# SeanNaren/deepspeech.pytorch

Hardware: NVIDIA H100
Metric: utterances/sec (train step, 161x1000 spectrogram) (higher is better)
Workload: dtype fp16-operands(rnn)+tf32(conv/fc)

## Files before the change

deepspeech.pytorch_b200/csrc/rnn_persistent_tc.cu:

```cuda
#include <cooperative_groups.h>
#include <cuda_fp16.h>
#include <dlfcn.h>
#include <stdlib.h>

#include "common.cuh"
#include "rnn_cells.cuh"
#include "rnn_common.cuh"
#include "tc_common.cuh"

namespace cg = cooperative_groups;

namespace ds2 {

namespace rp {
constexpr int UT = 16;
constexpr int MM = 64;
constexpr int BK = 32;
constexpr int STAGES = 8;
constexpr int THREADS = 288;
constexpr int A_BYTES = MM * 128;
constexpr long long SPIN_LIMIT = 4000000000LL;
}

struct PersistParams {
// ... 711 lines not shown
      uint32_t ph = 0;
      for (int step = 1; step < T; ++step) {
        const int t = d == 0 ? T - 1 - step : step;
        const int tn = d == 0 ? t + 1 : t - 1;
        for (int c = 0; c < NK; ++c) {
          mbar_wait(&empty[s], ph ^ 1);
          mbar_arrive_expect_tx(&full[s], tx_bytes);
          tma_load_2d(smem + s * STAGE_BYTES, &p.tmW[d], &full[s], c * BK, u0);
          if (c == 0) {
            grid_wait_counter(ctr, (unsigned int)p.NT * (unsigned int)step, p.err);
            fence_proxy_async_global();
            trace_stamp(p.trace, p.T, step, 0);
          }
          const int k0 = c * BK;
          if (RNN == DS2_RNN_GRU && k0 >= 2 * H)
            tma_load_2d(smem + s * STAGE_BYTES + A_BYTES, &p.tmV2[d], &full[s], k0 - 2 * H, tn * B);
          else
            tma_load_2d(smem + s * STAGE_BYTES + A_BYTES, &p.tmV[d], &full[s], d * GH + k0, tn * B);
          if (++s == STAGES) { s = 0; ph ^= 1; }
        }
      }
    }
  } else if (warp >= 4) {
    with_nch<4>(NB, [&](auto nch) {
      WgAcc<1, decltype(nch)::value> acc;
      {
        const uint64_t a_base = smem_desc_sw128(smem_u32(smem));
        const uint64_t b_base = smem_desc_sw128(smem_u32(smem + A_BYTES));
        const uint64_t stage_step = (uint64_t)(STAGE_BYTES >> 4);
        int s = 0;
        uint32_t ph = 0;
        for (int step = 1; step < T; ++step) {
          for (int c = 0; c < NK; ++c) {
            mbar_wait(&full[s], ph);
            if (c == 0 && lane == 0) trace_stamp(p.trace, p.T, step, 1);
            if (c == NK - 1 && lane == 0) trace_stamp(p.trace, p.T, step, 2);
            const uint64_t ad = a_base + (uint64_t)s * stage_step, bd = b_base + (uint64_t)s * stage_step;
            wg_mma4<false>(acc, ad, bd, c > 0);
            wg_release_all(&empty[s]);
            if (++s == STAGES) { s = 0; ph ^= 1; }
          }
          wg_publish(acc, acc_img, accum_bar);
        }
      }
    });
  } else {
    const int q = warp % 4;
    const int e = threadIdx.x;
    uint32_t acc_phase = 0;
    for (int step = 0; step < T; ++step) {
      const int t = d == 0 ? T - 1 - step : step;
      const int tp = d == 0 ? t - 1 : t + 1;
      const bool tp_in = tp >= 0 && tp < T;
      if (q == 0 && step > 0) {
        mbar_wait(accum_bar, acc_phase);
        if (lane == 0) trace_stamp(p.trace, p.T, step, 3);
        for (int cb = 0; cb < NB; cb += 32) {
          float acc[32];
          tmem_ld32(acc_img, acc_pitch(NB), (uint32_t)cb, acc);
          if (lane < UT) {
#pragma unroll
            for (int j = 0; j < 32; ++j)
              if (cb + j < B) ex[lane * NBp + cb + j] = acc[j];
          }
        }
      }
      if (step > 0) acc_phase ^= 1;
      named_bar_sync(1, 128);
      if (e == 0) trace_stamp(p.trace, p.T, step, 4);
      for (int pi = e; pi < UT * B; pi += 128) {
        const int ui = pi % UT, b = pi / UT;
        const bool valid = t < p.len[b];
        const bool pin = tp_in && (d == 0 || tp < p.len[b]);
        const size_t si = (((size_t)d * T + t) * B + b) * H + u0 + ui;
        const size_t sp = (((size_t)d * T + (tp_in ? tp : 0)) * B + b) * H + u0 + ui;
        float* gp = p.gates + (((size_t)t * B + b) * D + d) * GH + u0 + ui;
        if (!valid) {
#pragma unroll
          for (int g = 0; g < G; ++g) gp[g * H] = 0.f;
          if (RNN == DS2_RNN_GRU) p.aux[si] = 0.f;
        } else {
          float dh = p.dy[((size_t)t * B + b) * H + u0 + ui] + ex[ui * NBp + b];
          if (RNN == DS2_RNN_LSTM) {
            const float c_prev = pin ? p.aux[sp] : 0.f;
            LstmBwd r = lstm_cell_bwd(gp[0], gp[H], gp[2 * H], gp[3 * H], p.aux[si], c_prev, dh, cst[ui * NBp + b]);
            gp[0] = r.di; gp[H] = r.df; gp[2 * H] = r.dg; gp[3 * H] = r.d_o;
            cst[ui * NBp + b] = r.dc_prev;
          } else if (RNN == DS2_RNN_GRU) {
            const float h_prev = pin ? p.hseq[sp] : 0.f;
            dh += cst[ui * NBp + b];
            GruBwd r = gru_cell_bwd(gp[0], gp[H], gp[2 * H], p.aux[si], h_prev, dh);
            gp[0] = r.dr; gp[H] = r.dz; gp[2 * H] = r.dxn;
            p.aux[si] = r.dhn;
            cst[ui * NBp + b] = r.dh_prev;
          } else {
            const float h = p.hseq[si];
            gp[0] = dh * (1.f - h * h);
          }
        }
      }
      named_bar_sync(1, 128);
      if (e == 0) {
        fence_proxy_async_global();
        red_release(ctr, 1u);
        trace_stamp(p.trace, p.T, step, 5);
      }
    }
  }
  __syncthreads();
}

__device__ __forceinline__ uint32_t mapa_u32(uint32_t addr, uint32_t rank) {
  uint32_t r;
  asm volatile("mapa.shared::cluster.u32 %0, %1, %2;" : "=r"(r) : "r"(addr), "r"(rank));
  return r;
}
__device__ __forceinline__ float ld_dsmem(uint32_t addr) {
  float v;
  asm volatile("ld.shared::cluster.f32 %0, [%1];" : "=f"(v) : "r"(addr) : "memory");
  return v;
}
__device__ __forceinline__ void mbar_arrive_remote(uint32_t cluster_addr) {
  asm volatile("mbarrier.arrive.release.cluster.shared::cluster.b64 _, [%0];" ::"r"(cluster_addr) : "memory");
}
__device__ __forceinline__ void mbar_wait_cluster(uint64_t* bar, uint32_t parity, int* err) {
  uint32_t ok = 0, it = 0;
  long long t0 = 0;
  while (!ok) {
    asm volatile(
        "{\n\t.reg .pred p;\n\t"
        "mbarrier.try_wait.parity.acquire.cluster.shared::cta.b64 p, [%1], %2;\n\t"
        "selp.u32 %0, 1, 0, p;\n\t}"
        : "=r"(ok)
        : "r"(tc::smem_u32(bar)), "r"(parity)
        : "memory");
    if (!ok && (++it & 1023u) == 0) {
      if (t0 == 0) t0 = clock64();
      if (*(volatile int*)err) return;
      if (clock64() - t0 > rp::SPIN_LIMIT) { *(volatile int*)err = 1; return; }
    }
  }
}
__host__ __device__ constexpr int xt_cgs(int rows) { return (rows + rows / 8) * 4 + 4; }
__host__ __device__ constexpr int xt_slice(int rows, int nb) { return (nb / 4) * xt_cgs(rows); }
__device__ __forceinline__ int xt_off(int rows, int row, int col) {
  return (col >> 2) * xt_cgs(rows) + (row + (row >> 3)) * 4 + (col & 3);
}
__device__ __forceinline__ void st_async_v4(uint32_t cluster_addr, float a, float b, float c, float d, uint32_t cluster_bar) {
  asm volatile("st.async.weak.shared::cluster.mbarrier::complete_tx::bytes.v4.f32 [%0], {%1, %2, %3, %4}, [%5];" ::"r"(
                   cluster_addr),
               "f"(a), "f"(b), "f"(c), "f"(d), "r"(cluster_bar)
               : "memory");
}
__device__ __forceinline__ void bulk_load(void* smem_dst, const void* src, uint32_t bytes, uint64_t* bar) {
  asm volatile("cp.async.bulk.shared::cluster.global.mbarrier::complete_tx::bytes [%0], [%1], %2, [%3];" ::"r"(
                   tc::smem_u32(smem_dst)),
               "l"(src), "r"(bytes), "r"(tc::smem_u32(bar))
               : "memory");
}
__device__ __forceinline__ void cluster_sync_all() {
  asm volatile("barrier.cluster.arrive.release.aligned;\n\tbarrier.cluster.wait.acquire.aligned;" ::: "memory");
}

__device__ __forceinline__ __half to_half_sat(float v) {
  return __float2half_rn(fminf(fmaxf(v, -65000.f), 65000.f));
}
__device__ __forceinline__ int pow2_exp_for(unsigned int m_bits, int sx_prev) {
  if (m_bits == 0u || m_bits >= 0x7f800000u) return sx_prev;
  const int E = (int)((m_bits >> 23) & 0xffu);
  return max(-100, min(100, 134 - E));
}
__device__ __forceinline__ float pow2f(int ex) { return __int_as_float((ex + 127) << 23); }

template <int RNN, bool RES, int CL, int NKR_T = 0, bool XG = false>
__global__ void __launch_bounds__(rp::THREADS, 1) rnn_bwd_splitk_kernel(const __grid_constant__ PersistParams p) {
  using namespace rp;
  using namespace tc;
  static_assert(!XG || (RES && CL == 4), "the L2 exchange is built for the resident 4-CTA variant");
  constexpr int G = RNN == DS2_RNN_LSTM ? 4 : (RNN == DS2_RNN_GRU ? 3 : 1);
  constexpr int UM = UT * CL;
  constexpr int A_BYTES = UM * 128;
  extern __shared__ uint8_t smem_raw[];
  uint8_t* smem = smem_raw + ((1024u - (tc::smem_u32(smem_raw) & 1023u)) & 1023u);
  const int NB = p.NB, B = p.B, T = p.T, H = p.H, D = p.D;
  const int B_BYTES = NB * 128, STAGE_BYTES = A_BYTES + B_BYTES;
  const int NBp = NB + 1;
  const int NKR = NKR_T ? NKR_T : (G * H / CL) / 64;
  const int NG = grp_count(NKR);
  const int ring_bytes = RES ? NKR * STAGE_BYTES : STAGES * STAGE_BYTES;
  float* part = reinterpret_cast<float*>(smem + ring_bytes);
  float* cst = part + CL * xt_slice(UT, NB);
  int* lens_s = reinterpret_cast<int*>(cst + UT * NBp);
  unsigned int* cta_max = reinterpret_cast<unsigned int*>(lens_s + ((NB + 1) & ~1));
  uint64_t* full = reinterpret_cast<uint64_t*>(cta_max + 2);
  uint64_t* empty = full + (RES ? 32 : STAGES);
  uint64_t* accum_bar = empty + STAGES;
  uint64_t* part_bar = accum_bar + 1;
  float* acc_img = reinterpret_cast<float*>(part_bar + 1);

  const int warp = threadIdx.x / 32, lane = threadIdx.x % 32;
  const int ks = blockIdx.x % CL;
  const int cl = blockIdx.x / CL;
  const int NTc = H / UM;
  const int d = p.d0 + cl / NTc, ut = cl % NTc;
  const int GH = G * H;
  const int Kc = GH / CL, NK = Kc / BK;
  const int kbase = ks * Kc;
  const int u0 = ut * UM + ks * UT;
  unsigned int* ctr = p.bar + 32 * d;
  const unsigned int n_arrive = (unsigned int)(NTc * CL);
  const int ss = xt_slice(UT, NB);
  const int grp0 = (d * NTc + ut) * CL;
  auto xslot = [&](int cta, int src, int step) { return p.xbuf + ((size_t)(cta * CL + src) * 2 + (step & 1)) * ss; };

  if (warp == 0 && lane == 0) {
    tma_prefetch_desc(&p.tmW[d]);
    tma_prefetch_desc(&p.tmV[d]);
    for (int i = 0; i < (RES ? 32 : STAGES); ++i) mbar_init(&full[i], 1);
    for (int i = 0; i < STAGES; ++i) mbar_init(&empty[i], RES ? 1 : 128);
    mbar_init(accum_bar, 1);
    mbar_init(part_bar, XG ? 2 : 1);
    fence_barrier_init();
    cta_max[0] = 0u;
  }
  for (int i = threadIdx.x; i < UT * NBp; i += THREADS) cst[i] = 0.f;
  for (int i = threadIdx.x; i < NB; i += THREADS) lens_s[i] = i < B ? p.len[i] : 0;
  __syncthreads();
  if constexpr (!XG) cluster_sync_all();
  const uint32_t tx_bytes = (uint32_t)(UM * 128 + B * 128);

  if (warp == 8) {
    if (RES) {
      if (lane == 0) {
        mbar_arrive_expect_tx(&empty[0], (uint32_t)(NKR * UM * 128));
        for (int c = 0; c < NKR; ++c) tma_load_2d(smem + c * A_BYTES, &p.tmW[d], &empty[0], kbase + c * 64, ut * UM);
        uint8_t* vbuf = smem + NKR * A_BYTES;
        for (int step = 1; step < T; ++step) {
          const int t = d == 0 ? T - 1 - step : step;
          const int tn = d == 0 ? t + 1 : t - 1;
          grid_wait_counter(ctr, n_arrive * (unsigned int)step, p.err);
          fence_proxy_async_global();
          trace_stamp(p.trace, p.T, step, 0);
          const unsigned int gm = ld_relaxed(p.gmax + (size_t)d * (T + 1) + step);
          for (int g = 0; g < NG; ++g) {
            uint64_t* fb = full + g;
            const int c0 = grp_begin(g), c1 = min(NKR, grp_begin(g + 1));
            if (c1 == NKR) *(volatile unsigned int*)(cta_max + 1) = gm;
            if (p.box3) {
              mbar_arrive_expect_tx(fb, (uint32_t)(4 * B_BYTES));
              tma_load_3d(vbuf + c0 * B_BYTES, &p.tmV3[d], fb, 0, tn * B, (d * GH + kbase) / 64 + c0);
            } else {
              mbar_arrive_expect_tx(fb, (uint32_t)((c1 - c0) * B * 128));
              for (int c = c0; c < c1; ++c)
                tma_load_2d(vbuf + c * B_BYTES, &p.tmV[d], fb, d * GH + kbase + c * 64, tn * B);
            }
          }
          trace_stamp(p.trace, p.T, step, 1);
          if constexpr (XG) {
            grid_wait_counter(p.xcnt + grp0 + ks, (unsigned int)((CL - 1) * step), p.err);
            fence_proxy_async_global();
            mbar_arrive_expect_tx(part_bar, (uint32_t)((CL - 1) * ss * 4));
            for (int src = 0; src < CL; ++src)
              if (src != ks) bulk_load(part + src * ss, xslot(grp0 + ks, src, step), (uint32_t)(ss * 4), part_bar);
          }
        }
      }
    } else
    if (lane == 0) {
      int s = 0;
      uint32_t ph = 0;
      for (int step = 1; step < T; ++step) {
        const int t = d == 0 ? T - 1 - step : step;
        const int tn = d == 0 ? t + 1 : t - 1;
        for (int c = 0; c < NK; ++c) {
          mbar_wait(&empty[s], ph ^ 1);
          mbar_arrive_expect_tx(&full[s], tx_bytes);
          const int k0 = kbase + c * BK;
          tma_load_2d(smem + s * STAGE_BYTES, &p.tmW[d], &full[s], k0, ut * UM);
          if (c == 0) {
            grid_wait_counter(ctr, n_arrive * (unsigned int)step, p.err);
            fence_proxy_async_global();
            trace_stamp(p.trace, p.T, step, 0);
          }
          if (RNN == DS2_RNN_GRU && k0 >= 2 * H)
            tma_load_2d(smem + s * STAGE_BYTES + A_BYTES, &p.tmV2[d], &full[s], k0 - 2 * H, tn * B);
          else
            tma_load_2d(smem + s * STAGE_BYTES + A_BYTES, &p.tmV[d], &full[s], d * GH + k0, tn * B);
          if (++s == STAGES) { s = 0; ph ^= 1; }
        }
      }
    }
  } else if (warp >= 4) {
    with_nch<UM == 64 ? 4 : 2>(NB, [&](auto nch) {
      WgAcc<UM / 64, decltype(nch)::value> acc;
      if (RES) {
        {
          const uint64_t a_base = warp_uniform(smem_desc_sw128(smem_u32(smem)));
          const uint64_t b_base = warp_uniform(smem_desc_sw128(smem_u32(smem + NKR * A_BYTES)));
          const uint64_t a_step = (uint64_t)(A_BYTES >> 4), b_step = (uint64_t)(B_BYTES >> 4);
          mbar_wait(&empty[0], 0);
          uint32_t ph = 0;
          for (int step = 1; step < T; ++step) {
            if constexpr (NKR_T > 0) {
              constexpr int NGT = (NKR_T + 3) / 4;
  #pragma unroll
              for (int g = 0; g < NGT; ++g) {
                mbar_wait(full + g, ph);
                if (g == 0 && lane == 0) trace_stamp(p.trace, p.T, step, 2);
                if (g == NGT - 1 && lane == 0) trace_stamp(p.trace, p.T, step, 3);
  #pragma unroll
                for (int c = 4 * g; c < (4 * g + 4 < NKR_T ? 4 * g + 4 : NKR_T); ++c) {
                  const uint64_t ad = a_base + (uint64_t)c * a_step, bd = b_base + (uint64_t)c * b_step;
                  wg_mma4<true>(acc, ad, bd, c > 0);
                }
              }
            } else {
              for (int g = 0; g < NG; ++g) {
                mbar_wait(full + g, ph);
                if (g == 0 && lane == 0) trace_stamp(p.trace, p.T, step, 2);
                const int c0 = grp_begin(g), c1 = min(NKR, grp_begin(g + 1));
                if (c1 == NKR && lane == 0) trace_stamp(p.trace, p.T, step, 3);
                for (int c = c0; c < c1; ++c) {
                  const uint64_t ad = a_base + (uint64_t)c * a_step, bd = b_base + (uint64_t)c * b_step;
                  wg_mma4<true>(acc, ad, bd, c > 0);
                }
              }
            }
            wg_publish(acc, acc_img, accum_bar);
            if (lane == 0) trace_stamp(p.trace, p.T, step, 4);
            ph ^= 1;
          }
        }
      } else
      {
        const uint64_t a_base = smem_desc_sw128(smem_u32(smem));
        const uint64_t b_base = smem_desc_sw128(smem_u32(smem + A_BYTES));
        const uint64_t stage_step = (uint64_t)(STAGE_BYTES >> 4);
        int s = 0;
        uint32_t ph = 0;
        for (int step = 1; step < T; ++step) {
          for (int c = 0; c < NK; ++c) {
            mbar_wait(&full[s], ph);
            if (c == 0 && lane == 0) trace_stamp(p.trace, p.T, step, 1);
            if (c == NK - 1 && lane == 0) trace_stamp(p.trace, p.T, step, 2);
            const uint64_t ad = a_base + (uint64_t)s * stage_step, bd = b_base + (uint64_t)s * stage_step;
            wg_mma4<false>(acc, ad, bd, c > 0);
            wg_release_all(&empty[s]);
            if (++s == STAGES) { s = 0; ph ^= 1; }
          }
          wg_publish(acc, acc_img, accum_bar);
        }
      }
    });
  } else {
    const int q = warp % 4;
    const int e = threadIdx.x;
    const int ul = lane & 15, half = lane >> 4;
    uint32_t acc_phase = 0, part_phase = 0;
    const int dst_cta = CL == 4 ? q : 2 * q + half;
    const uint32_t dst_row = XG ? 0u : mapa_u32(smem_u32(part), (uint32_t)dst_cta) + (uint32_t)(ks * ss * 4);
    const uint32_t dst_bar = XG ? 0u : mapa_u32(smem_u32(part_bar), (uint32_t)dst_cta);
    const uint32_t part_tx = (uint32_t)(CL * UT * NB * 4);
    float bsum[5][4];
#pragma unroll
    for (int i = 0; i < 5; ++i)
#pragma unroll
      for (int j = 0; j < 4; ++j) bsum[i][j] = 0.f;
    int sx_prev = 0, sx_cur = 0;
    if (RES) sx_cur = pow2_exp_for(__ldg(p.dymax + (d == 0 ? T - 1 : 0)), 0);
    float s_cur = pow2f(sx_cur), inv_prev = 1.f;
    const float nscale = (RES && p.dgn16) ? __ldg(p.nscale) : 1.f;
    for (int step = 0; step < T; ++step) {
      const int t = d == 0 ? T - 1 - step : step;
      const int tp = d == 0 ? t - 1 : t + 1;
      const bool tp_in = tp >= 0 && tp < T;
      float lmax = 0.f;
      const unsigned int dym = RES ? __ldg(p.dymax + t) : 0u;
      constexpr int NPF = 4;
      const bool single = B <= 32;
      const int uq = 4 * (e & 3), b_own = e >> 2;
      auto ld4 = [](const float* src, float (&v)[NPF]) {
        const float4 x = *reinterpret_cast<const float4*>(src);
        v[0] = x.x; v[1] = x.y; v[2] = x.z; v[3] = x.w;
      };
      auto load_coefs = [&](int b, float (&k)[6][NPF], float (&dyv)[NPF], bool& valid) {
#pragma unroll
        for (int i = 0; i < 6; ++i)
#pragma unroll
          for (int j = 0; j < NPF; ++j) k[i][j] = 0.f;
#pragma unroll
        for (int j = 0; j < NPF; ++j) dyv[j] = 0.f;
        valid = b < B && t < lens_s[b < B ? b : 0];
        if (!valid) return;
        const bool pin = tp_in && (d == 0 || tp < lens_s[b]);
        const size_t si = (((size_t)d * T + t) * B + b) * H + u0 + uq;
        const size_t sp = (((size_t)d * T + (tp_in ? tp : 0)) * B + b) * H + u0 + uq;
        const float* gp = p.gates + (((size_t)t * B + b) * D + d) * GH + u0 + uq;
        ld4(p.dy + ((size_t)t * B + b) * H + u0 + uq, dyv);
        if (RNN == DS2_RNN_LSTM) {
          float gi[NPF], gf[NPF], gg[NPF], go[NPF], c[NPF], c_prev[NPF] = {0.f, 0.f, 0.f, 0.f}, tc[NPF];
          ld4(gp, gi); ld4(gp + H, gf); ld4(gp + 2 * H, gg); ld4(gp + 3 * H, go);
          ld4(p.aux + si, c);
          if (pin) ld4(p.aux + sp, c_prev);
#pragma unroll
          for (int j = 0; j < NPF; ++j) tc[j] = ex2_ftz(-2.f * LOG2E * c[j]);
#pragma unroll
          for (int j = 0; j < NPF; ++j) tc[j] = fmaf(2.f, rcp_ftz(1.f + tc[j]), -1.f);
#pragma unroll
          for (int j = 0; j < NPF; ++j) {
            k[0][j] = go[j] * (1.f - tc[j] * tc[j]); k[1][j] = tc[j] * go[j] * (1.f - go[j]);
            k[2][j] = gg[j] * gi[j] * (1.f - gi[j]); k[3][j] = c_prev[j] * gf[j] * (1.f - gf[j]);
            k[4][j] = gi[j] * (1.f - gg[j] * gg[j]); k[5][j] = gf[j];
          }
        } else if (RNN == DS2_RNN_GRU) {
          float r[NPF], z[NPF], n[NPF], hn[NPF], h_prev[NPF] = {0.f, 0.f, 0.f, 0.f};
          ld4(gp, r); ld4(gp + H, z); ld4(gp + 2 * H, n);
          ld4(p.aux + si, hn);
          if (pin) ld4(p.hseq + sp, h_prev);
#pragma unroll
          for (int j = 0; j < NPF; ++j) {
            const float cn = (1.f - z[j]) * (1.f - n[j] * n[j]);
            k[0][j] = cn * hn[j] * r[j] * (1.f - r[j]); k[1][j] = (h_prev[j] - n[j]) * z[j] * (1.f - z[j]);
            k[2][j] = cn; k[3][j] = cn * r[j]; k[4][j] = z[j];
          }
        } else {
          float hv[NPF];
          ld4(p.hseq + si, hv);
#pragma unroll
          for (int j = 0; j < NPF; ++j) k[0][j] = 1.f - hv[j] * hv[j];
        }
      };
      float kc[6][NPF], pdy[NPF];
      bool pvalid = false;
      if (single) load_coefs(b_own, kc, pdy, pvalid);
      if (step > 0) {
        if (!XG && e == 0) mbar_arrive_expect_tx(part_bar, part_tx);
        mbar_wait(accum_bar, acc_phase);
        if (RES) {
          const unsigned int gm = *(volatile unsigned int*)(cta_max + 1);
          sx_prev = sx_cur;
          sx_cur = pow2_exp_for(max(gm, dym), sx_prev);
          s_cur = pow2f(sx_cur);
          inv_prev = pow2f(-sx_prev);
        }
        if (e == 0) trace_stamp(p.trace, p.T, step, 5);
        float* const xdst = XG ? (q == ks ? part + ks * ss : xslot(grp0 + q, ks, step)) : nullptr;
        for (int cb = 0; cb < NB; cb += 32) {
          float acc[32];
          tmem_ld32(acc_img, acc_pitch(NB), ((uint32_t)(q * 32) << 16) + (uint32_t)cb, acc);
          if (CL == 4) {
            float v[16];
#pragma unroll
            for (int j = 0; j < 16; ++j) {
              const float hi = __shfl_sync(0xffffffffu, acc[16 + j], ul);
              v[j] = half ? hi : acc[j];
            }
#pragma unroll
            for (int i = 0; i < 4; ++i) {
              const int c0 = cb + half * 16 + 4 * i;
              if (c0 >= NB) continue;
              if constexpr (XG) {
                *reinterpret_cast<float4*>(xdst + xt_off(UT, ul, c0)) = make_float4(v[4 * i], v[4 * i + 1], v[4 * i + 2], v[4 * i + 3]);
              } else {
                st_async_v4(dst_row + (uint32_t)(xt_off(UT, ul, c0) * 4), v[4 * i], v[4 * i + 1], v[4 * i + 2], v[4 * i + 3], dst_bar);
              }
            }
          } else {
#pragma unroll
            for (int i = 0; i < 8; ++i) {
              const int c0 = cb + 4 * i;
              if (c0 < NB)
                st_async_v4(dst_row + (uint32_t)(xt_off(UT, ul, c0) * 4), acc[4 * i], acc[4 * i + 1], acc[4 * i + 2], acc[4 * i + 3], dst_bar);
            }
          }
        }
        acc_phase ^= 1;
        if (e == 0) trace_stamp(p.trace, p.T, step, 6);
        if constexpr (XG) {
          __syncwarp();
          if (lane == 0) {
            if (q == ks) {
              mbar_arrive(part_bar);
            } else {
              fence_proxy_async_global();
              red_release(p.xcnt + grp0 + q, 1u);
            }
          }
        }
        mbar_wait_cluster(part_bar, part_phase, p.err);
        part_phase ^= 1;
      }
      if (e == 0) trace_stamp(p.trace, p.T, step, 7);
      auto st_h4 = [&](__half* dst, const float (&v)[NPF]) {
        const __half2 lo = __halves2half2(to_half_sat(v[0] * s_cur), to_half_sat(v[1] * s_cur));
        const __half2 hi = __halves2half2(to_half_sat(v[2] * s_cur), to_half_sat(v[3] * s_cur));
        uint2 pk;
        pk.x = *reinterpret_cast<const unsigned int*>(&lo);
        pk.y = *reinterpret_cast<const unsigned int*>(&hi);
        *reinterpret_cast<uint2*>(dst) = pk;
      };
      auto finish4 = [&](int b, const float (&k)[6][NPF], const float (&dyv)[NPF], bool valid, float (&o)[5][NPF]) {
#pragma unroll
        for (int i = 0; i < 5; ++i)
#pragma unroll
          for (int j = 0; j < NPF; ++j) o[i][j] = 0.f;
        if (b >= B) return;
        __half* hp16 = RES ? p.dg16 + (((size_t)t * B + b) * D + d) * GH + u0 + uq : nullptr;
        if (!valid) {
          if (RES) {
#pragma unroll
            for (int g = 0; g < G; ++g) *reinterpret_cast<uint2*>(hp16 + g * H) = make_uint2(0u, 0u);
          }
          return;
        }
        float dh[NPF];
#pragma unroll
        for (int j = 0; j < NPF; ++j) {
          float rec = 0.f;
          if (step > 0) {
            const float* pr = part + xt_off(UT, uq + j, b);
            rec = (pr[0] + pr[ss]) + (pr[2 * ss] + pr[3 * ss]);
            if (CL == 8) rec += (pr[4 * ss] + pr[5 * ss]) + (pr[6 * ss] + pr[7 * ss]);
          }
          dh[j] = dyv[j] + (RES ? rec * inv_prev : rec);
        }
        if (RNN == DS2_RNN_LSTM) {
#pragma unroll
          for (int j = 0; j < NPF; ++j) {
            const int ci = (uq + j) * NBp + b;
            const float dc = fmaf(dh[j], k[0][j], cst[ci]);
            o[0][j] = dc * k[2][j]; o[1][j] = dc * k[3][j]; o[2][j] = dc * k[4][j]; o[3][j] = dh[j] * k[1][j];
            cst[ci] = dc * k[5][j];
            lmax = fmaxf(lmax, fmaxf(fmaxf(fabsf(o[0][j]), fabsf(o[1][j])), fmaxf(fabsf(o[2][j]), fabsf(o[3][j]))));
          }
          if (RES) {
#pragma unroll
            for (int g = 0; g < 4; ++g) st_h4(hp16 + g * H, o[g]);
          }
        } else if (RNN == DS2_RNN_GRU) {
#pragma unroll
          for (int j = 0; j < NPF; ++j) {
            const int ci = (uq + j) * NBp + b;
            const float dht = dh[j] + cst[ci];
            o[0][j] = dht * k[0][j]; o[1][j] = dht * k[1][j]; o[2][j] = dht * k[2][j]; o[4][j] = dht * k[3][j];
            cst[ci] = dht * k[4][j];
            lmax = fmaxf(lmax, fmaxf(fabsf(o[0][j]), fmaxf(fabsf(o[1][j]), fabsf(o[4][j]))));
          }
          if (RES) {
            st_h4(hp16, o[0]); st_h4(hp16 + H, o[1]);
            st_h4(hp16 + 2 * H, o[4]);
          }
        } else {
#pragma unroll
          for (int j = 0; j < NPF; ++j) {
            o[0][j] = dh[j] * k[0][j];
            lmax = fmaxf(lmax, fabsf(o[0][j]));
          }
          if (RES) st_h4(hp16, o[0]);
        }
      };
      auto st4 = [](float* dst, const float (&v)[NPF]) {
        *reinterpret_cast<float4*>(dst) = make_float4(v[0], v[1], v[2], v[3]);
      };
      auto store_dg = [&](int b, const float (&o)[5][NPF]) {
#pragma unroll
        for (int i = 0; i < 5; ++i)
#pragma unroll
          for (int j = 0; j < NPF; ++j) bsum[i][j] += o[i][j];
        float* gp = p.gates + (((size_t)t * B + b) * D + d) * GH + u0 + uq;
#pragma unroll
        for (int g = 0; g < G; ++g) st4(gp + g * H, o[g]);
        if (RNN == DS2_RNN_GRU) st4(p.aux + (((size_t)d * T + t) * B + b) * H + u0 + uq, o[4]);
        if (RES && p.dgn16) {
          const size_t TBs = (size_t)T * B, col = (size_t)t * B + b;
          __half* r16 = p.dgn16 + (col * D + d) * GH + u0 + uq;
          __half* t16 = p.dgn16T + ((size_t)d * GH + u0 + uq) * TBs + col;
#pragma unroll
          for (int g = 0; g < G; ++g) {
            __half h[NPF];
#pragma unroll
            for (int j = 0; j < NPF; ++j) {
              h[j] = to_half_sat(o[g][j] * nscale);
              t16[((size_t)g * H + j) * TBs] = h[j];
            }
            const __half2 lo = __halves2half2(h[0], h[1]), hi = __halves2half2(h[2], h[3]);
            uint2 pk;
            pk.x = *reinterpret_cast<const unsigned int*>(&lo);
            pk.y = *reinterpret_cast<const unsigned int*>(&hi);
            *reinterpret_cast<uint2*>(r16 + g * H) = pk;
          }
          if (RNN == DS2_RNN_GRU) {
            __half* a16 = p.auxn16T + ((size_t)d * H + u0 + uq) * TBs + col;
#pragma unroll
            for (int j = 0; j < NPF; ++j) a16[(size_t)j * TBs] = to_half_sat(o[4][j] * nscale);
          }
        }
      };
      const bool defer = RES && p.defer && single;
      float sv[5][NPF];
      if (single) {
        finish4(b_own, kc, pdy, pvalid, sv);
        if (!defer && b_own < B) store_dg(b_own, sv);
      } else {
        for (int b = b_own; b < B; b += 32) {
          load_coefs(b, kc, pdy, pvalid);
          finish4(b, kc, pdy, pvalid, sv);
          store_dg(b, sv);
        }
      }
      if (RES) {
#pragma unroll
        for (int o = 16; o > 0; o >>= 1) lmax = fmaxf(lmax, __shfl_xor_sync(0xffffffffu, lmax, o));
        if (lane == 0) atomicMax(cta_max, __float_as_uint(lmax));
      }
      if (e == 0) trace_stamp(p.trace, p.T, step, 8);
      named_bar_sync(1, 128);
      if (e == 0) {
        trace_stamp(p.trace, p.T, step, 9);
        if (RES) {
          atomicMax(p.gmax + (size_t)d * (T + 1) + step + 1, cta_max[0]);
          cta_max[0] = 0u;
        }
        fence_proxy_async_global();
        trace_stamp(p.trace, p.T, step, 10);
        red_release(ctr, 1u);
        trace_stamp(p.trace, p.T, step, 11);
        trace_stamp_ns(p.trace, p.T, step, 12);
      }
      if (defer) {
        if (b_own < B) store_dg(b_own, sv);
        if (e == 0) trace_stamp(p.trace, p.T, step, 13);
      }
    }
    if (p.dbias[d]) {
      named_bar_sync(1, 128);
      float* red = part;
#pragma unroll
      for (int i = 0; i < 5; ++i) {
#pragma unroll
        for (int j = 0; j < 4; ++j) {
          float v = bsum[i][j];
          v += __shfl_xor_sync(0xffffffffu, v, 4);
          v += __shfl_xor_sync(0xffffffffu, v, 8);
// ... 280 lines not shown
            for (int g = 0; g < 2; ++g)
#pragma unroll
              for (int k = 0; k < 4; ++k) a[g][k] = rcp_ftz(1.f + a[g][k]);
#pragma unroll
            for (int k = 0; k < 4; ++k) nv[k] = ex2_ftz(-2.f * LOG2E * fmaf(a[0][k], hn[k], pre[2][k]));
#pragma unroll
            for (int k = 0; k < 4; ++k) nv[k] = rcp_ftz(1.f + nv[k]);
#pragma unroll
            for (int k = 0; k < 4; ++k) {
              const float nval = valid[k] ? fmaf(2.f, nv[k], -1.f) : 0.f;
              hval[k] = valid[k] ? fmaf(a[1][k], cp[k] - nval, nval) : 0.f;
              if (valid[k]) cp[k] = hval[k];
              o[0][k] = valid[k] ? a[0][k] : 0.f; o[1][k] = valid[k] ? a[1][k] : 0.f; o[2][k] = nval; o[3][k] = 0.f;
              o[4][k] = valid[k] ? hn[k] : 0.f;
            }
          }
#pragma unroll
          for (int k = 0; k < 4; ++k) o[5][k] = hval[k];
        };
        const int bs = fwd_store_col(tid);
        const int us = u0 + 4 * (tid >> 5);
        auto store4 = [&](int c, const float (&o)[6][4]) {
          const int b = 32 * c + bs;
          if (b < B) {
            const size_t so = (((size_t)d * T + t) * B + b) * H + us;
            float* gp = p.gates + (((size_t)t * B + b) * D + d) * GH + us;
            *reinterpret_cast<float4*>(p.aux + so) = make_float4(o[4][0], o[4][1], o[4][2], o[4][3]);
            if (p.training) {
#pragma unroll
              for (int g = 0; g < G; ++g)
                *reinterpret_cast<float4*>(gp + (size_t)g * H) = make_float4(o[g][0], o[g][1], o[g][2], o[g][3]);
            }
            *reinterpret_cast<float4*>(p.hseq + so) = make_float4(o[5][0], o[5][1], o[5][2], o[5][3]);
          }
        };
        float sv[NCH][6][4];
#pragma unroll
        for (int c = 0; c < NCH; ++c) {
          if (NCH > 1) load_gx(c);
          float o[6][4];
          cell4(c, gx[c], s[c], cs[c], o);
#pragma unroll
          for (int q = 0; q < 6; ++q)
            if (q < G || q >= 4) fwd_units4(o[q], sv[c][q]);
          const int b = 32 * c + bs;
          if (b < B) {
            float h4[4] = {sv[c][5][0], sv[c][5][1], sv[c][5][2], sv[c][5][3]};
            if constexpr (ST) {
              if (d == 1 && t >= p.len[b]) {
#pragma unroll
                for (int j = 0; j < 4; ++j) h4[j] = p.h0 ? p.h0[((size_t)B + b) * H + us + j] : 0.f;
              }
            }
            const __half2 lo = __floats2half2_rn(h4[0], h4[1]), hi = __floats2half2_rn(h4[2], h4[3]);
            uint2 pk;
            pk.x = *reinterpret_cast<const unsigned int*>(&lo);
            pk.y = *reinterpret_cast<const unsigned int*>(&hi);
            *reinterpret_cast<uint2*>(p.h16 + (((size_t)d * T + t) * B + b) * H + us) = pk;
          }
          if (!defer) store4(c, sv[c]);
        }
        if (tid == 0) trace_stamp(p.trace, p.T, step, 8);
        named_bar_sync(1, 128);
        if (tid == 0) {
          trace_stamp(p.trace, p.T, step, 9);
          fence_proxy_async_global();
          trace_stamp(p.trace, p.T, step, 10);
          red_release(ctr, 1u);
          trace_stamp(p.trace, p.T, step, 11);
          trace_stamp_ns(p.trace, p.T, step, 12);
        }
        if (defer) {
          named_bar_sync(4, 256);
#pragma unroll
          for (int q = 0; q < 6; ++q)
            if (q < G || q >= 4) stage[q * 128 + tid] = make_float4(sv[0][q][0], sv[0][q][1], sv[0][q][2], sv[0][q][3]);
          asm volatile("bar.arrive 3, 256;" ::: "memory");
        }
      }
    });
  } else if (stage_saves) {
    const int tid = threadIdx.x;
    const int b = fwd_store_col(tid), us = u0 + 4 * (tid >> 5);
    for (int step = 0; step < T; ++step) {
      const int t = d == 0 ? step : T - 1 - step;
      asm volatile("bar.arrive 4, 256;" ::: "memory");
      named_bar_sync(3, 256);
      if (b < B) {
        const size_t so = (((size_t)d * T + t) * B + b) * H + us;
        float* gp = p.gates + (((size_t)t * B + b) * D + d) * GH + us;
        *reinterpret_cast<float4*>(p.aux + so) = stage[4 * 128 + tid];
        if (p.training) {
#pragma unroll
          for (int g = 0; g < G; ++g) *reinterpret_cast<float4*>(gp + (size_t)g * H) = stage[g * 128 + tid];
        }
        *reinterpret_cast<float4*>(p.hseq + so) = stage[5 * 128 + tid];
      }
      if (tid == 0) trace_stamp(p.trace, p.T, step, 13);
    }
  }
  __syncthreads();
  cluster_sync_all();
}

template <int RNN, int NKR_T = 0>
__global__ void __launch_bounds__(rp::THREADS, 1) rnn_fwd_splitk_kernel(const __grid_constant__ PersistParams p) {
  fwd_splitk_sweep<RNN, NKR_T, false>(p);
}
constexpr int FWD_SPLITK_MAX_NKR = 10;
template <int RNN, int NKR_T>
__global__ void __launch_bounds__(rp::THREADS, 1) rnn_fwd_splitk_state_kernel(const __grid_constant__ PersistParams p) {
  static_assert(NKR_T == 1 || NKR_T == 5 || NKR_T == 8 || NKR_T == 9, "an ST chunk count that compiles without spills");
  fwd_splitk_sweep<RNN, NKR_T, true>(p);
}
template <int RNN>
static const SweepKernel fwd_splitk_state_kernels[FWD_SPLITK_MAX_NKR] = {
    rnn_fwd_splitk_state_kernel<RNN, 1>, nullptr, nullptr, nullptr, rnn_fwd_splitk_state_kernel<RNN, 5>, nullptr,
    nullptr, rnn_fwd_splitk_state_kernel<RNN, 8>, rnn_fwd_splitk_state_kernel<RNN, 9>, nullptr};

static size_t fwd_splitk_smem_bytes(int NB, int H, bool defer) {
  return 1024 + (size_t)(H / 128) * (128 * 128 + (size_t)NB * 128) + (size_t)64 * NB * sizeof(float) +
         (defer && NB == 32 ? 6 * 128 * 16 : 0) + 10 * sizeof(uint64_t) + 64;
}

template <int RNN>
static int launch_fwd_splitk(const SeqArgs& a, void* ws, size_t ws_bytes, cudaStream_t st) {
  constexpr int G = RNN == DS2_RNN_LSTM ? 4 : 3;
  if (a.H % 128 != 0 || a.H / 128 > 32) return 1;
  if (!vec_ok(a.gates, a.hseq, a.aux) || !a.aux) return 1;
  if (ws_bytes < res_ws_bytes(G, a.T, a.B, a.H, a.D)) return 1;
  PersistParams p = sweep_params(a, 32, "DS2_TRACE_FWD", ws);
  if (p.NB > 64) return 1;
  const size_t smem = one_cta_per_sm(fwd_splitk_smem_bytes(p.NB, a.H, p.defer));
  if (smem > 227 * 1024) return 1;
  const bool state = a.h0 || a.c0;
  const int nkr = a.H / 128;
  if (state && (nkr > FWD_SPLITK_MAX_NKR || !fwd_splitk_state_kernels<RNN>[nkr - 1])) return 1;
  const SweepKernel kern = state ? fwd_splitk_state_kernels<RNN>[nkr - 1]
                                 : (a.H == 1024 ? rnn_fwd_splitk_kernel<RNN, 8> : rnn_fwd_splitk_kernel<RNN, 0>);
  static DeviceOnce attr_once;
  const SweepKernel* sk = fwd_splitk_state_kernels<RNN>;
  if (int rc = opt_in_smem(attr_once, {rnn_fwd_splitk_kernel<RNN, 8>, rnn_fwd_splitk_kernel<RNN, 0>, sk[0], sk[4], sk[7],
                                       sk[8]}))
    return rc;
  const int fit = cluster_fit(kern, 2, a.D * p.NT * 2, smem, st);
  return launch_sweep(kern, 2, p.NT * 2, smem, fit, true, 4096, "split-K forward sweep", "the 16-unit kernel", p, st,
                      [&] { return f16_weight_maps(a, p, ws, a.H / 128, st, true, state); });
}

static size_t splitk_smem_bytes(int NB, int CL) {
  using namespace rp;
  size_t NBp = NB + 1;
  return 1024 + (size_t)STAGES * ((size_t)UT * CL * 128 + (size_t)NB * 128) +
         ((size_t)CL * xt_slice(UT, NB) + UT * NBp + NB + 16) * sizeof(float) + (2 * STAGES + 3) * sizeof(uint64_t) + 64 + tc::acc_image_bytes(NB);
}

__global__ void absmax_rows_kernel(size_t n, const float* __restrict__ x, unsigned int* __restrict__ out) {
  __shared__ float red[8];
  const float* row = x + (size_t)blockIdx.x * n;
  float m = 0.f;
  for (size_t i = threadIdx.x * 4; i + 3 < n; i += blockDim.x * 4) {
    const float4 v = *reinterpret_cast<const float4*>(row + i);
    m = fmaxf(m, fmaxf(fmaxf(fabsf(v.x), fabsf(v.y)), fmaxf(fabsf(v.z), fabsf(v.w))));
  }
  for (size_t i = (n & ~(size_t)3) + threadIdx.x; i < n; i += blockDim.x) m = fmaxf(m, fabsf(row[i]));
#pragma unroll
  for (int o = 16; o > 0; o >>= 1) m = fmaxf(m, __shfl_xor_sync(0xffffffffu, m, o));
  if (threadIdx.x % 32 == 0) red[threadIdx.x / 32] = m;
  __syncthreads();
  if (threadIdx.x == 0) {
    for (int w = 1; w < (int)(blockDim.x / 32); ++w) m = fmaxf(m, red[w]);
    out[blockIdx.x] = __float_as_uint(m);
  }
}

static size_t splitk_res_smem_bytes(int NB, int Kc, int CL) {
  using namespace rp;
  size_t NBp = NB + 1;
  return 1024 + (size_t)(Kc / 64) * ((size_t)UT * CL * 128 + (size_t)NB * 128) +
         ((size_t)CL * xt_slice(UT, NB) + UT * NBp + NB + 16) * sizeof(float) + (32 + STAGES + 3) * sizeof(uint64_t) + 64 + tc::acc_image_bytes(NB);
}
constexpr size_t XCNT_OFFSET = 1024;
constexpr int XCNT_MAX = (4096 - (int)XCNT_OFFSET) / 4;
static size_t splitk_xbuf_bytes(int B, int H, int D) {
  return (size_t)D * (H / 16) * 4 * 2 * xt_slice(rp::UT, (B + 31) / 32 * 32) * sizeof(float);
}
static size_t splitk_res_ws_bytes(int G, int T, int B, int H, int D) {
  const size_t GH = (size_t)G * H;
  return 4096 + align_up((size_t)D * (T + 1) * 4, 256) + align_up((size_t)T * 4, 256) +
         align_up((size_t)D * H * GH * 2, 256) + align_up((size_t)T * B * D * GH * 2, 256) +
         align_up(splitk_xbuf_bytes(B, H, D), 256);
}

template <int RNN, int CL>
static int launch_bwd_splitk_resident(const SeqArgs& a, void* ws, size_t ws_bytes, cudaStream_t st) {
  using namespace rp;
  const int G = RNN == DS2_RNN_LSTM ? 4 : (RNN == DS2_RNN_GRU ? 3 : 1);
  const int GH = G * a.H;
  constexpr int UM = UT * CL;
  if (a.H % UM != 0 || GH % CL != 0 || (GH / CL) % 64 != 0 || (GH / CL) / 64 > 120) return 1;
  if (CL == 8 && ((a.B + 7) / 8 * 8) % 16 != 0) return 1;
  if (!vec_ok(a.gates, a.hseq, a.aux, a.dy)) return 1;
  if (ws_bytes < splitk_res_ws_bytes(G, a.T, a.B, a.H, a.D)) return 1;
  PersistParams p = sweep_params(a, UM, "DS2_TRACE_BWD", ws);
  if (p.NB > (CL == 8 ? 64 : 128)) return 1;
  for (int d = 0; d < a.D; ++d) { p.dbias[d] = a.dbias[d]; p.dbias_hn[d] = a.dbias_hn[d]; }
  if (a.f16_dg && a.f16_dgT && a.f16_scale && (RNN != DS2_RNN_GRU || a.f16_auxT)) {
    p.dgn16 = static_cast<__half*>(a.f16_dg);
    p.dgn16T = static_cast<__half*>(a.f16_dgT);
    p.auxn16T = static_cast<__half*>(a.f16_auxT);
    p.nscale = a.f16_scale;
  }
  char* base = static_cast<char*>(ws);
  size_t off = 4096;
  p.gmax = reinterpret_cast<unsigned int*>(base + off); off += align_up((size_t)a.D * (a.T + 1) * 4, 256);
  p.dymax = reinterpret_cast<unsigned int*>(base + off); off += align_up((size_t)a.T * 4, 256);
  __half* wT16 = reinterpret_cast<__half*>(base + off); off += align_up((size_t)a.D * a.H * GH * 2, 256);
  p.dg16 = reinterpret_cast<__half*>(base + off); off += align_up((size_t)a.T * a.B * a.D * GH * 2, 256);
  p.xbuf = reinterpret_cast<float*>(base + off);
  p.xcnt = reinterpret_cast<unsigned int*>(base + XCNT_OFFSET);
  const size_t smem = one_cta_per_sm(splitk_res_smem_bytes(p.NB, GH / CL, CL));
  if (smem > 227 * 1024) return 1;
  const char* xe = getenv("DS2_SPLITK_XCHG");
  const bool force_cluster = xe && !strcmp(xe, "cluster"), force_global = xe && !strcmp(xe, "global");
  if (force_global && CL != 4) return 1;
  constexpr int NKU = (G * 1024 / CL) / 64;
  SweepKernel kern = a.H == 1024 ? rnn_bwd_splitk_kernel<RNN, true, CL, NKU> : rnn_bwd_splitk_kernel<RNN, true, CL, 0>;
  static DeviceOnce attr_once;
  int rc;
  if constexpr (CL == 4)
    rc = opt_in_smem(attr_once, {rnn_bwd_splitk_kernel<RNN, true, CL, NKU>, rnn_bwd_splitk_kernel<RNN, true, CL, 0>,
                                 rnn_bwd_splitk_kernel<RNN, true, CL, NKU, true>, rnn_bwd_splitk_kernel<RNN, true, CL, 0, true>});
  else
    rc = opt_in_smem(attr_once, {rnn_bwd_splitk_kernel<RNN, true, CL, NKU>, rnn_bwd_splitk_kernel<RNN, true, CL, 0>});
  if (rc) return rc;
  const int grid = a.D * p.NT * CL;
  int cluster = CL;
  int fit = cluster_fit(kern, CL, grid, smem, st);
  if (fit < 0) return 1;
  if (force_global || (fit < grid && !force_cluster)) {
    if constexpr (CL == 4) {
      const SweepKernel kern_xg =
          a.H == 1024 ? rnn_bwd_splitk_kernel<RNN, true, CL, NKU, true> : rnn_bwd_splitk_kernel<RNN, true, CL, 0, true>;
      int resident = 0;
      if ((rc = coop_fit(kern_xg, smem, &resident))) return rc;
      if (grid <= XCNT_MAX && (resident >= grid || force_global)) {
        kern = kern_xg;
        cluster = 1;
        fit = resident;
      }
    }
    if (force_global && cluster != 1) return 1;
  }
  rc = launch_sweep(kern, cluster, p.NT * CL, smem, fit, CL != 8, 4096 + align_up((size_t)a.D * (a.T + 1) * 4, 256),
                    "resident split-K backward sweep", CL == 8 ? nullptr : "a slower variant", p, st, [&]() -> int {
    const size_t wn = (size_t)a.H * GH;
    const bool cached = a.w_hhT16[0] && (a.D == 1 || a.w_hhT16[1]);
    if (!cached) {
      int mrc = materialize_w_hh(a, st);
      if (mrc) return mrc;
    }
    for (int d = 0; d < a.D; ++d) {
      const __half* wsrc = static_cast<const __half*>(a.w_hhT16[d]);
      if (!cached) {
        DS2_LAUNCH(f32_to_f16_kernel, 132 * 4, 256, 0, st, wn, a.w_hh[d], wT16 + (size_t)d * wn);
        wsrc = wT16 + (size_t)d * wn;
      }
      int trc = make_tmap_f16(&p.tmW[d], wsrc, 2, GH, a.H, 1, (size_t)GH, 0, 64, UM, 1);
      if (trc) return trc;
      trc = make_tmap_f16(&p.tmV[d], p.dg16, 2, a.D * GH, a.T * a.B, 1, (size_t)a.D * GH, 0, 64, a.B, 1);
      if (trc) return trc;
      p.box3 = ((GH / CL) / 64) % 4 == 0;
      if (p.box3) {
        trc = make_tmap_f16(&p.tmV3[d], p.dg16, 3, 64, a.T * a.B, a.D * GH / 64, (size_t)a.D * GH, 64, 64, p.NB, 4);
        if (trc) return trc;
      }
    }
    DS2_LAUNCH(absmax_rows_kernel, a.T, 256, 0, st, (size_t)a.B * a.H, a.dy, p.dymax);
    return DS2_OK;
  });
  if (rc != DS2_OK) return rc;
  if (a.dbias_done && a.dbias[0]) *a.dbias_done = 1;
  if (a.f16_done && p.dgn16) *a.f16_done = 1;
  return DS2_OK;
}

template <int RNN, int CL>
static int launch_bwd_splitk(const SeqArgs& a, void* ws, size_t ws_bytes, cudaStream_t st) {
  using namespace rp;
  const int G = RNN == DS2_RNN_LSTM ? 4 : (RNN == DS2_RNN_GRU ? 3 : 1);
  const int GH = G * a.H;
  if (!getenv("DS2_NO_RESIDENT")) {
    int rc = launch_bwd_splitk_resident<RNN, CL>(a, ws, ws_bytes, st);
    if (rc != 1) return rc;
  }
  constexpr int UM = UT * CL;
  if (a.H % UM != 0 || (GH / CL) % BK != 0 || GH % CL != 0) return 1;
  { int mrc = materialize_w_hh(a, st); if (mrc) return mrc; }
  if (CL == 8 && ((a.B + 7) / 8 * 8) % 16 != 0) return 1;
  if (!vec_ok(a.gates, a.hseq, a.aux, a.dy)) return 1;
  PersistParams p = sweep_params(a, UM, "DS2_TRACE_BWD", ws);
  if (p.NB > (CL == 8 ? 64 : 128)) return 1;
  if (ws_bytes < 4096) return 1;
  const size_t smem = one_cta_per_sm(splitk_smem_bytes(p.NB, CL));
  if (smem > 227 * 1024) return 1;
  const SweepKernel kern = rnn_bwd_splitk_kernel<RNN, false, CL>;
  static DeviceOnce attr_once;
  if (int rc = opt_in_smem(attr_once, {kern})) return rc;
  const int fit = cluster_fit(kern, CL, a.D * p.NT * CL, smem, st);
  return launch_sweep(kern, CL, p.NT * CL, smem, fit, CL != 8, 4096, "split-K backward sweep", nullptr, p, st, [&] {
    for (int d = 0; d < a.D; ++d) {
      int rc = make_tmap_2d(&p.tmW[d], a.w_hh[d], a.H, GH, GH, UM, BK);
      if (rc) return rc;
      rc = make_tmap_2d(&p.tmV[d], a.gates, a.T * a.B, a.D * GH, a.D * GH, a.B, BK);
      if (rc) return rc;
      if (RNN == DS2_RNN_GRU) {
        rc = make_tmap_2d(&p.tmV2[d], a.aux + (size_t)d * a.T * a.B * a.H, a.T * a.B, a.H, a.H, a.B, BK);
        if (rc) return rc;
      }
    }
    return 0;
  });
}

template <int RNN>
static int launch_bwd(const SeqArgs& a, void* ws, size_t ws_bytes, cudaStream_t st) {
  using namespace rp;
  const int G = RNN == DS2_RNN_LSTM ? 4 : (RNN == DS2_RNN_GRU ? 3 : 1);
  const int GH = G * a.H;
  { int mrc = materialize_w_hh(a, st); if (mrc) return mrc; }
  PersistParams p = sweep_params(a, UT, "DS2_TRACE_BWD", ws);
  if (p.NB > 128) return 1;
  if (ws_bytes < 4096) return 1;
// ... 48 lines not shown
```

Before: 629.2.

## Scatter split-K partials directly from MMA warps to cluster peers

```diff
diff --git a/deepspeech.pytorch_b200/csrc/rnn_persistent_tc.cu b/deepspeech.pytorch_b200/csrc/rnn_persistent_tc.cu
--- a/deepspeech.pytorch_b200/csrc/rnn_persistent_tc.cu
+++ b/deepspeech.pytorch_b200/csrc/rnn_persistent_tc.cu
@@ -887,6 +887,12 @@
                "f"(a), "f"(b), "f"(c), "f"(d), "r"(cluster_bar)
                : "memory");
 }
+__device__ __forceinline__ void st_async_v2(uint32_t cluster_addr, float a, float b, uint32_t cluster_bar) {
+  asm volatile("st.async.weak.shared::cluster.mbarrier::complete_tx::bytes.v2.f32 [%0], {%1, %2}, [%3];" ::"r"(
+                   cluster_addr),
+               "f"(a), "f"(b), "r"(cluster_bar)
+               : "memory");
+}
 __device__ __forceinline__ void bulk_load(void* smem_dst, const void* src, uint32_t bytes, uint64_t* bar) {
   asm volatile("cp.async.bulk.shared::cluster.global.mbarrier::complete_tx::bytes [%0], [%1], %2, [%3];" ::"r"(
                    tc::smem_u32(smem_dst)),
@@ -929,9 +935,7 @@
   unsigned int* cta_max = reinterpret_cast<unsigned int*>(lens_s + ((NB + 1) & ~1));
   uint64_t* full = reinterpret_cast<uint64_t*>(cta_max + 2);
   uint64_t* empty = full + (RES ? 32 : STAGES);
-  uint64_t* accum_bar = empty + STAGES;
-  uint64_t* part_bar = accum_bar + 1;
-  float* acc_img = reinterpret_cast<float*>(part_bar + 1);
+  uint64_t* part_bar = empty + STAGES;
 
   const int warp = threadIdx.x / 32, lane = threadIdx.x % 32;
   const int ks = blockIdx.x % CL;
@@ -953,8 +957,7 @@
     tma_prefetch_desc(&p.tmV[d]);
     for (int i = 0; i < (RES ? 32 : STAGES); ++i) mbar_init(&full[i], 1);
     for (int i = 0; i < STAGES; ++i) mbar_init(&empty[i], RES ? 1 : 128);
-    mbar_init(accum_bar, 1);
-    mbar_init(part_bar, XG ? 2 : 1);
+    mbar_init(part_bar, 2);
     fence_barrier_init();
     cta_max[0] = 0u;
   }
@@ -1027,7 +1030,54 @@
     }
   } else if (warp >= 4) {
     with_nch<UM == 64 ? 4 : 2>(NB, [&](auto nch) {
-      WgAcc<UM / 64, decltype(nch)::value> acc;
+      constexpr int MH = UM / 64, NCH = decltype(nch)::value;
+      WgAcc<MH, NCH> acc;
+      const int wq = warp - 4;
+      auto dst_of = [&](int h) { return CL == 4 ? wq : 4 * h + wq; };
+      uint32_t dst_tile[MH], dst_bar[MH];
+#pragma unroll
+      for (int h = 0; h < MH; ++h) {
+        dst_tile[h] = XG ? 0u : mapa_u32(smem_u32(part + ks * ss), (uint32_t)dst_of(h));
+        dst_bar[h] = XG ? 0u : mapa_u32(smem_u32(part_bar), (uint32_t)dst_of(h));
+      }
+      const int lane_off = xt_off(UT, lane >> 2, 2 * (lane & 3));
+      auto send = [&](int step) {
+        wg_commit();
+        wg_wait<0>();
+        if (lane == 0) trace_stamp(p.trace, p.T, step, 4);
+#pragma unroll
+        for (int h = 0; h < MH; ++h) {
+          const int dst = dst_of(h);
+          float* const own = part + ks * ss + lane_off;
+          float* const xdst = XG ? xslot(grp0 + dst, ks, step) + lane_off : own;
+#pragma unroll
+          for (int c = 0; c < NCH; ++c)
+#pragma unroll
+            for (int i = 0; i < 4; ++i)
+#pragma unroll
+              for (int hh = 0; hh < 2; ++hh) {
+                const int off = (8 * c + 2 * i) * xt_cgs(UT) + 36 * hh;
+                const float v0 = acc.r[h][c][4 * i + 2 * hh], v1 = acc.r[h][c][4 * i + 2 * hh + 1];
+                if (dst == ks) *reinterpret_cast<float2*>(own + off) = make_float2(v0, v1);
+                else if constexpr (XG) *reinterpret_cast<float2*>(xdst + off) = make_float2(v0, v1);
+                else st_async_v2(dst_tile[h] + (uint32_t)((lane_off + off) * 4), v0, v1, dst_bar[h]);
+              }
+        }
+        __syncwarp();
+        if (lane == 0) {
+          trace_stamp(p.trace, p.T, step, 6);
+#pragma unroll
+          for (int h = 0; h < MH; ++h) {
+            const int dst = dst_of(h);
+            if (dst == ks) {
+              mbar_arrive(part_bar);
+            } else if constexpr (XG) {
+              fence_proxy_async_global();
+              red_release(p.xcnt + grp0 + dst, 1u);
+            }
+          }
+        }
+      };
       if (RES) {
         {
           const uint64_t a_base = warp_uniform(smem_desc_sw128(smem_u32(smem)));
@@ -1061,8 +1111,7 @@
                 }
               }
             }
-            wg_publish(acc, acc_img, accum_bar);
-            if (lane == 0) trace_stamp(p.trace, p.T, step, 4);
+            send(step);
             ph ^= 1;
           }
         }
@@ -1083,19 +1132,15 @@
             wg_release_all(&empty[s]);
             if (++s == STAGES) { s = 0; ph ^= 1; }
           }
-          wg_publish(acc, acc_img, accum_bar);
+          send(step);
         }
       }
     });
   } else {
     const int q = warp % 4;
     const int e = threadIdx.x;
-    const int ul = lane & 15, half = lane >> 4;
-    uint32_t acc_phase = 0, part_phase = 0;
-    const int dst_cta = CL == 4 ? q : 2 * q + half;
-    const uint32_t dst_row = XG ? 0u : mapa_u32(smem_u32(part), (uint32_t)dst_cta) + (uint32_t)(ks * ss * 4);
-    const uint32_t dst_bar = XG ? 0u : mapa_u32(smem_u32(part_bar), (uint32_t)dst_cta);
-    const uint32_t part_tx = (uint32_t)(CL * UT * NB * 4);
+    uint32_t part_phase = 0;
+    const uint32_t part_tx = (uint32_t)((CL - 1) * UT * NB * 4);
     float bsum[5][4];
 #pragma unroll
     for (int i = 0; i < 5; ++i)
@@ -1170,7 +1215,8 @@
       if (single) load_coefs(b_own, kc, pdy, pvalid);
       if (step > 0) {
         if (!XG && e == 0) mbar_arrive_expect_tx(part_bar, part_tx);
-        mbar_wait(accum_bar, acc_phase);
+        mbar_wait_cluster(part_bar, part_phase, p.err);
+        part_phase ^= 1;
         if (RES) {
           const unsigned int gm = *(volatile unsigned int*)(cta_max + 1);
           sx_prev = sx_cur;
@@ -1178,52 +1224,6 @@
           s_cur = pow2f(sx_cur);
           inv_prev = pow2f(-sx_prev);
         }
-        if (e == 0) trace_stamp(p.trace, p.T, step, 5);
-        float* const xdst = XG ? (q == ks ? part + ks * ss : xslot(grp0 + q, ks, step)) : nullptr;
-        for (int cb = 0; cb < NB; cb += 32) {
-          float acc[32];
-          tmem_ld32(acc_img, acc_pitch(NB), ((uint32_t)(q * 32) << 16) + (uint32_t)cb, acc);
-          if (CL == 4) {
-            float v[16];
-#pragma unroll
-            for (int j = 0; j < 16; ++j) {
-              const float hi = __shfl_sync(0xffffffffu, acc[16 + j], ul);
-              v[j] = half ? hi : acc[j];
-            }
-#pragma unroll
-            for (int i = 0; i < 4; ++i) {
-              const int c0 = cb + half * 16 + 4 * i;
-              if (c0 >= NB) continue;
-              if constexpr (XG) {
-                *reinterpret_cast<float4*>(xdst + xt_off(UT, ul, c0)) = make_float4(v[4 * i], v[4 * i + 1], v[4 * i + 2], v[4 * i + 3]);
-              } else {
-                st_async_v4(dst_row + (uint32_t)(xt_off(UT, ul, c0) * 4), v[4 * i], v[4 * i + 1], v[4 * i + 2], v[4 * i + 3], dst_bar);
-              }
-            }
-          } else {
-#pragma unroll
-            for (int i = 0; i < 8; ++i) {
-              const int c0 = cb + 4 * i;
-              if (c0 < NB)
-                st_async_v4(dst_row + (uint32_t)(xt_off(UT, ul, c0) * 4), acc[4 * i], acc[4 * i + 1], acc[4 * i + 2], acc[4 * i + 3], dst_bar);
-            }
-          }
-        }
-        acc_phase ^= 1;
-        if (e == 0) trace_stamp(p.trace, p.T, step, 6);
-        if constexpr (XG) {
-          __syncwarp();
-          if (lane == 0) {
-            if (q == ks) {
-              mbar_arrive(part_bar);
-            } else {
-              fence_proxy_async_global();
-              red_release(p.xcnt + grp0 + q, 1u);
-            }
-          }
-        }
-        mbar_wait_cluster(part_bar, part_phase, p.err);
-        part_phase ^= 1;
       }
       if (e == 0) trace_stamp(p.trace, p.T, step, 7);
       auto st_h4 = [&](__half* dst, const float (&v)[NPF]) {
@@ -1810,7 +1810,7 @@
   using namespace rp;
   size_t NBp = NB + 1;
   return 1024 + (size_t)STAGES * ((size_t)UT * CL * 128 + (size_t)NB * 128) +
-         ((size_t)CL * xt_slice(UT, NB) + UT * NBp + NB + 16) * sizeof(float) + (2 * STAGES + 3) * sizeof(uint64_t) + 64 + tc::acc_image_bytes(NB);
+         ((size_t)CL * xt_slice(UT, NB) + UT * NBp + NB + 16) * sizeof(float) + (2 * STAGES + 2) * sizeof(uint64_t) + 64;
 }
 
 __global__ void absmax_rows_kernel(size_t n, const float* __restrict__ x, unsigned int* __restrict__ out) {
@@ -1836,7 +1836,7 @@
   using namespace rp;
   size_t NBp = NB + 1;
   return 1024 + (size_t)(Kc / 64) * ((size_t)UT * CL * 128 + (size_t)NB * 128) +
-         ((size_t)CL * xt_slice(UT, NB) + UT * NBp + NB + 16) * sizeof(float) + (32 + STAGES + 3) * sizeof(uint64_t) + 64 + tc::acc_image_bytes(NB);
+         ((size_t)CL * xt_slice(UT, NB) + UT * NBp + NB + 16) * sizeof(float) + (32 + STAGES + 2) * sizeof(uint64_t) + 64;
 }
 constexpr size_t XCNT_OFFSET = 1024;
 constexpr int XCNT_MAX = (4096 - (int)XCNT_OFFSET) / 4;
```

Result: faster. 638.6 (median of 6 runs) (+1.5%).
